# kyleliang919/distributed-lion-pytorch

Measured on AMD Instinct MI355X. Metric: tokens/sec + all-reduce bytes/step, GPT-2 CLM at 1/2/4/8 MI355X, higher is better.
Workload: dtype bf16; 1 GPU; model=gpt2 (124.4M params), trainable_params=124439808, base_weights=bf16, global_batch=160, task=clm, gradient_checkpointing=False, micro_batch=20, grad_accum=8, seq_len=1024, parallelism=dp1, optimizer=distributed Lion (majority vote), lr 0.0001, wd 0.1, exchange=a2a, impl=native

## Files before the change

distributed_lion_pytorch_amd/csrc/bindings.cpp:

```cpp
#include <ATen/ATen.h>
#include <c10/core/DeviceGuard.h>
#include <c10/hip/HIPStream.h>
#include <torch/library.h>

#include <hip/hip_runtime.h>

#include <cstdlib>
#include <string>
#include <vector>

#include "kernels.h"

namespace dlion {
enum class Layout : int { NT = 0, NN = 1, TN = 2, TT = 3 };
bool lt_gemm(const void* a, int64_t lda, const void* b, int64_t ldb, void* c, int64_t ldc, const void* bias,
             int64_t M, int64_t N, int64_t K, int epi, int device, hipStream_t s, Layout lay, bool accumulate);
}

namespace {

using at::Tensor;

void check_dev(const Tensor& t, const char* name) {
  TORCH_CHECK(t.is_cuda(), "dlion: ", name, " must be a GPU (HIP) tensor");
// ... 579 lines not shown
  return y;
}

void rope_(const Tensor& x, const Tensor& cos, const Tensor& sin, bool inverse) {
  TORCH_CHECK(x.dim() == 4 && x.is_cuda() && x.scalar_type() == at::kBFloat16, "dlion rope_: x must be bf16 [B, T, H, D]");
  const int64_t B = x.size(0), T = x.size(1), H = x.size(2), D = x.size(3);
  TORCH_CHECK(x.stride(3) == 1 && x.stride(2) == D && (B == 1 || x.stride(0) == T * x.stride(1)) &&
                  x.stride(1) % 8 == 0 && reinterpret_cast<uintptr_t>(x.data_ptr()) % 16 == 0 && D % 8 == 0,
              "dlion rope_: x must have contiguous heads and a uniform, 16-byte aligned token stride");
  for (const Tensor* t : {&cos, &sin})
    TORCH_CHECK(t->is_cuda() && t->scalar_type() == at::kBFloat16 && t->is_contiguous() && t->dim() == 2 &&
                    t->size(0) >= T && t->size(1) == D,
                "dlion rope_: cos/sin must be contiguous bf16 [>=T, D]");
  const c10::DeviceGuard dg(x.device());
  check_hip(dlion::launch_rope(x.data_ptr(), cos.data_ptr(), sin.data_ptr(), x.data_ptr(), B * T,
                               static_cast<int>(T), static_cast<int>(H), static_cast<int>(D), inverse, x.stride(1),
                               x.stride(1), cur_stream()),
            "rope_");
}

void check_gemm_operand(const Tensor& t, const char* name) {
  TORCH_CHECK(t.is_cuda() && t.scalar_type() == at::kBFloat16 && t.dim() == 2 && t.stride(1) == 1,
              "dlion gemm: ", name, " must be a 2-D bf16 GPU tensor with unit column stride");
  TORCH_CHECK(t.stride(0) % 8 == 0 && reinterpret_cast<uintptr_t>(t.data_ptr()) % 16 == 0,
              "dlion gemm: ", name, " rows must be 16-byte aligned");
}

bool gemm_nt_supported(const Tensor& a, const Tensor& b) {
  return a.dim() == 2 && b.dim() == 2 && a.size(1) == b.size(1) && a.size(1) % 128 == 0 && b.size(0) % 8 == 0 &&
         a.size(0) * a.stride(0) < (1ll << 31) && b.size(0) * b.stride(0) < (1ll << 31);
}

void gemm_nt_launch(const Tensor& a, const Tensor& b, const Tensor& c, const Tensor* bias, const Tensor* aux,
                    int64_t epi, const Tensor* part = nullptr) {
  check_gemm_operand(a, "a");
  check_gemm_operand(b, "b");
  check_gemm_operand(c, "out");
  TORCH_CHECK(gemm_nt_supported(a, b), "dlion gemm: unsupported shape a=", a.sizes(), " b=", b.sizes(),
              " (needs K % 128 == 0, N % 8 == 0)");
  TORCH_CHECK(c.size(0) == a.size(0) && c.size(1) == b.size(0), "dlion gemm: output shape mismatch");
  if (bias) {
    TORCH_CHECK(bias->is_cuda() && bias->scalar_type() == at::kBFloat16 && bias->is_contiguous() &&
                    bias->numel() == b.size(0),
                "dlion gemm: bias must be a contiguous bf16 [N] tensor");
  }
  if (aux) {
    check_gemm_operand(*aux, "aux");
    TORCH_CHECK(aux->size(0) == c.size(0) && aux->size(1) == c.size(1), "dlion gemm: aux must match the output shape");
  }
  if (part) {
    TORCH_CHECK(part->is_cuda() && part->scalar_type() == at::kFloat && part->is_contiguous() &&
                    part->size(0) == 2 * ((a.size(0) + 255) / 256) && part->size(1) == b.size(0),
                "dlion gemm: part must be fp32 [2 * ceil(M / 256), N]");
  }
  const c10::DeviceGuard g(a.device());
  check_hip(dlion::launch_gemm_nt(a.data_ptr(), static_cast<int>(a.stride(0)), b.data_ptr(),
                                  static_cast<int>(b.stride(0)), c.data_ptr(), static_cast<int>(c.stride(0)),
                                  bias ? bias->data_ptr() : nullptr, aux ? aux->data_ptr() : nullptr,
                                  aux ? static_cast<int>(aux->stride(0)) : 0, static_cast<int>(a.size(0)),
                                  static_cast<int>(b.size(0)), static_cast<int>(a.size(1)), static_cast<int>(epi),
                                  part ? part->data_ptr<float>() : nullptr, cur_stream()),
            "gemm_nt");
}

Tensor gemm_nt(const Tensor& a, const Tensor& b, const std::optional<Tensor>& bias) {
  auto c = at::empty({a.size(0), b.size(0)}, a.options());
  gemm_nt_launch(a, b, c, bias.has_value() ? &*bias : nullptr, nullptr, bias.has_value() ? 1 : 0);
  return c;
}

void gemm_nt_out(const Tensor& a, const Tensor& b, const std::optional<Tensor>& bias, const Tensor& out) {
  gemm_nt_launch(a, b, out, bias.has_value() ? &*bias : nullptr, nullptr, bias.has_value() ? 1 : 0);
}

std::tuple<Tensor, Tensor> gemm_nt_gelu(const Tensor& a, const Tensor& b, const Tensor& bias, bool exact) {
  auto h = at::empty({a.size(0), b.size(0)}, a.options());
  auto z = at::empty_like(h);
  gemm_nt_launch(a, b, h, &bias, &z, exact ? 3 : 2);
  return {h, z};
}

bool lt_gemm_nt(const Tensor& a, const Tensor& b, const std::optional<Tensor>& bias, int64_t epi, const Tensor& out) {
  check_gemm_operand(a, "a");
  check_gemm_operand(b, "b");
  check_gemm_operand(out, "out");
  TORCH_CHECK(epi >= 0 && epi <= 2, "dlion lt_gemm: bad epilogue ", epi);
  TORCH_CHECK(a.size(1) == b.size(1) && out.size(0) == a.size(0) && out.size(1) == b.size(0),
              "dlion lt_gemm: shape mismatch a=", a.sizes(), " b=", b.sizes(), " out=", out.sizes());
  TORCH_CHECK(bias.has_value() == (epi != 0), "dlion lt_gemm: epilogue ", epi, epi ? " needs" : " takes no", " bias");
  if (bias.has_value()) {
    TORCH_CHECK(bias->is_cuda() && bias->scalar_type() == at::kBFloat16 && bias->is_contiguous() &&
                    bias->numel() == b.size(0),
                "dlion lt_gemm: bias must be a contiguous bf16 [N] tensor");
  }
  const c10::DeviceGuard g(a.device());
// ... 106 lines not shown
    TORCH_CHECK(sid.has_value() && perm.has_value() && sid->numel() == n && perm->numel() == n &&
                    sid->scalar_type() == at::kLong && perm->scalar_type() == at::kLong && sid->is_contiguous() &&
                    perm->is_contiguous(),
                "dlion embed: the token gradient needs sorted ids and their permutation (int64 [n])");
    V = dwte->size(0);
  }
  if (dwpe.has_value()) {
    check_bf16_contig(*dwpe, "dwpe");
    TORCH_CHECK(dwpe->size(-1) == C && dwpe->size(0) >= T, "dlion embed: dwpe must be [>= T, C]");
  }
  const c10::DeviceGuard g(dx.device());
  const auto dp = drop_params(p);
  check_hip(dlion::launch_embed_bwd(dx.data_ptr(), dwte.has_value() ? sid->data_ptr<int64_t>() : nullptr,
                                    dwte.has_value() ? perm->data_ptr<int64_t>() : nullptr,
                                    dwte.has_value() ? dwte->data_ptr() : nullptr,
                                    dwpe.has_value() ? dwpe->data_ptr() : nullptr, n, static_cast<int>(C),
                                    static_cast<int>(T), V, pos_accumulate ? 1 : 0, static_cast<uint32_t>(seed),
                                    dp.first, dp.second, cur_stream()),
            "embed_bwd");
}

void scale_acc_(const Tensor& x, const Tensor& s, const Tensor& y, bool accumulate) {
  check_bf16_contig(x, "x");
  check_bf16_contig(y, "y");
  check_dev(s, "s");
  TORCH_CHECK(s.scalar_type() == at::kFloat && s.numel() >= 1, "dlion scale_acc: s must be float32");
  TORCH_CHECK(x.numel() == y.numel() && x.numel() % 8 == 0, "dlion scale_acc: size mismatch / numel % 8 != 0");
  const c10::DeviceGuard g(x.device());
  check_hip(dlion::launch_scale_acc(x.data_ptr(), s.data_ptr<float>(), y.data_ptr(), x.numel(), accumulate ? 1 : 0,
                                    cur_stream()),
            "scale_acc");
}

Tensor gemm_nt_stamped(const Tensor& a, const Tensor& b, const Tensor& stamps) {
  check_gemm_operand(a, "a");
  check_gemm_operand(b, "b");
  TORCH_CHECK(gemm_nt_supported(a, b), "dlion gemm: unsupported shape");
  const int64_t blocks = ((a.size(0) + 255) / 256) * ((b.size(0) + 255) / 256);
  TORCH_CHECK(stamps.is_cuda() && stamps.scalar_type() == at::kLong && stamps.is_contiguous() &&
                  stamps.numel() >= blocks * 8,
              "dlion gemm: stamps must be int64 [blocks, 8]");
  auto c = at::empty({a.size(0), b.size(0)}, a.options());
  const c10::DeviceGuard g(a.device());
  check_hip(dlion::launch_gemm_nt_stamped(a.data_ptr(), static_cast<int>(a.stride(0)), b.data_ptr(),
                                          static_cast<int>(b.stride(0)), c.data_ptr(), static_cast<int>(c.stride(0)),
                                          static_cast<int>(a.size(0)), static_cast<int>(b.size(0)),
                                          static_cast<int>(a.size(1)),
                                          reinterpret_cast<unsigned long long*>(stamps.data_ptr<int64_t>()),
                                          cur_stream()),
            "gemm_nt_stamped");
  return c;
}

std::tuple<Tensor, Tensor> gemm_nt_gelu_d(const Tensor& a, const Tensor& b, const Tensor& bias, bool exact) {
  auto h = at::empty({a.size(0), b.size(0)}, a.options());
  auto d = at::empty({a.size(0), b.size(0)}, a.options());
  gemm_nt_launch(a, b, h, &bias, &d, exact ? 7 : 6);
  return {h, d};
}

std::tuple<Tensor, Tensor> gemm_nt_dmul(const Tensor& a, const Tensor& b, const Tensor& d) {
  auto dz = at::empty({a.size(0), b.size(0)}, a.options());
  auto part = at::empty({2 * ((a.size(0) + 255) / 256), b.size(0)}, a.options().dtype(at::kFloat));
  gemm_nt_launch(a, b, dz, nullptr, &d, 8, &part);
  return {dz, part};
}

std::tuple<Tensor, Tensor> gemm_nt_dgelu(const Tensor& a, const Tensor& b, const Tensor& bias, const Tensor& z,
                                         bool exact) {
  auto dz = at::empty({a.size(0), b.size(0)}, a.options());
  auto part = at::empty({2 * ((a.size(0) + 255) / 256), b.size(0)}, a.options().dtype(at::kFloat));
  gemm_nt_launch(a, b, dz, &bias, &z, exact ? 5 : 4, &part);
  return {dz, part};
}

void gemm_tn_check_launch(at::TensorList P, at::TensorList Q, int64_t splits, const Tensor& out, bool accumulate) {
  TORCH_CHECK(!P.empty() && P.size() == Q.size() && P.size() <= 16, "dlion gemm_tn: 1..16 segment pairs");
  const int64_t rows = P[0].size(0), M = P[0].size(1), N = Q[0].size(1);
  const int64_t ldp = P[0].stride(0), ldq = Q[0].stride(0);
  std::vector<const void*> pp, qq;
  for (size_t i = 0; i < P.size(); ++i) {
    for (const Tensor* t : {&P[i], &Q[i]}) {
// ... 162 lines not shown
}

void dequant4_t_(const Tensor& q, const Tensor& absmax, const Tensor& code, const Tensor& out) {
  check_dev(q, "q");
  check_dev(absmax, "absmax");
  check_dev(code, "code");
  TORCH_CHECK(out.is_cuda() && out.dim() == 2 && out.stride(1) == 1 && out.element_size() == 2,
              "dlion dequant4_t: out must be a 2-D 16-bit GPU view with unit column stride");
  const int64_t K = out.size(0), N = out.size(1);
  TORCH_CHECK(q.scalar_type() == at::kByte && q.numel() * 2 == N * K && absmax.numel() * 64 == N * K &&
                  code.numel() == 16 && code.scalar_type() == at::kFloat,
              "dlion dequant4_t: q / absmax do not match out");
  const c10::DeviceGuard g(out.device());
  check_hip(dlion::launch_dequant4_t(dtype_code(out.scalar_type()), q.data_ptr<uint8_t>(), absmax.data_ptr<float>(),
                                     code.data_ptr<float>(), out.data_ptr(), static_cast<int>(N), static_cast<int>(K),
                                     out.stride(0), cur_stream()),
            "dequant4_t");
}
}

TORCH_LIBRARY(dlion, m) {
  m.def("dequant4_t_(Tensor q, Tensor absmax, Tensor code, Tensor(a!) out) -> ()");
  m.def("transpose_pad(Tensor x, int rows_out=-1) -> Tensor");
  m.def("quant4(Tensor w, Tensor code) -> (Tensor, Tensor)");
  m.def("dequant4_(Tensor q, Tensor absmax, Tensor code, Tensor(a!) out) -> ()");
  m.def("gemm_tn(Tensor[] P, Tensor[] Q, int splits) -> Tensor");
  m.def("gemm_tn_(Tensor[] P, Tensor[] Q, Tensor(a!) out, bool accumulate) -> ()");
  m.def("lora_rows(Tensor x, Tensor w, float scale, float p, int seed) -> Tensor");
  m.def("lora_up(Tensor o, Tensor u, Tensor b, float s) -> Tensor");
  m.def("lora_cols(Tensor g, Tensor y, Tensor? a, float yscale, float p, int seed) -> (Tensor, Tensor)");
  m.def("gemm_nt_dgelu(Tensor a, Tensor b, Tensor bias, Tensor z, bool exact) -> (Tensor, Tensor)");
  m.def("gemm_nt_gelu_d(Tensor a, Tensor b, Tensor bias, bool exact) -> (Tensor, Tensor)");
  m.def("gemm_nt_dmul(Tensor a, Tensor b, Tensor d) -> (Tensor, Tensor)");
  m.def("gemm_nt_stamped(Tensor a, Tensor b, Tensor(a!) stamps) -> Tensor");
  m.def("embed_fwd(Tensor ids, Tensor wte, Tensor wpe, float p, int seed, Tensor(a!)? err=None) -> Tensor");
  m.def("index_check_(Tensor ids, int hi, int ignore, Tensor(a!) err, int code) -> ()");
  m.def(
      "embed_bwd_(Tensor dx, Tensor? sid, Tensor? perm, Tensor(a!)? dwte, Tensor(b!)? dwpe, int T, bool pos_accumulate,"
      " float p, int seed) -> ()");
  m.def("scale_acc_(Tensor x, Tensor s, Tensor(a!) y, bool accumulate) -> ()");
  m.def("lt_gemm_nt(Tensor a, Tensor b, Tensor? bias, int epi, Tensor(a!) out) -> bool");
  m.def("lt_gemm_nn(Tensor a, Tensor b, Tensor(a!) out) -> bool");
  m.def("lt_gemm_tn(Tensor a, Tensor b, Tensor(a!) out, bool accumulate) -> bool");
  m.def("lt_gemm_nt_acc(Tensor a, Tensor b, Tensor(a!) out, bool accumulate) -> bool");
  m.def("lt_gemm_layout(Tensor a, Tensor b, Tensor(a!) out, int layout, bool accumulate) -> bool");
  m.def("gemm_nt(Tensor a, Tensor b, Tensor? bias) -> Tensor");
  m.def("gemm_nt_out(Tensor a, Tensor b, Tensor? bias, Tensor(a!) out) -> ()");
  m.def("gemm_nt_gelu(Tensor a, Tensor b, Tensor bias, bool exact) -> (Tensor, Tensor)");
  m.def("swiglu_fwd(Tensor g, Tensor u) -> Tensor");
  m.def("swiglu_bwd(Tensor dh, Tensor g, Tensor u) -> (Tensor, Tensor)");
  m.def("swiglu_bwd_fused(Tensor dh, Tensor g, Tensor u) -> Tensor");
  m.def("swiglu_bwd_fused_t(Tensor dh, Tensor g, Tensor u) -> (Tensor, Tensor)");
  m.def("swiglu_fwd_t(Tensor g, Tensor u) -> (Tensor, Tensor)");
  m.def("rope(Tensor x, Tensor cos, Tensor sin, bool inverse) -> Tensor");
  m.def("rope_(Tensor(a!) x, Tensor cos, Tensor sin, bool inverse) -> ()");
  m.def(
      "add_norm_fwd(Tensor x, Tensor? y, Tensor? bias, Tensor gamma, Tensor? beta, float eps, bool rms, float p,"
      " int seed) -> (Tensor, Tensor, Tensor, Tensor)");
  m.def(
      "add_norm_bwd(Tensor dh, Tensor? dxo_in, Tensor xo, Tensor gamma, Tensor mean, Tensor rstd, bool rms,"
      " float p, int seed, bool want_dy, int parts) -> (Tensor, Tensor, Tensor)");
  m.def("bias_gelu_fwd(Tensor z, Tensor b, bool exact) -> Tensor");
  m.def("bias_gelu_bwd(Tensor dh, Tensor z, Tensor b, bool exact, int parts) -> (Tensor, Tensor)");
  m.def("sum_partials(Tensor part) -> Tensor");
  m.def("sum_partials_acc_(Tensor part, Tensor(a!) out) -> ()");
  m.def("sum_partials_scaled_(Tensor part, Tensor s, Tensor(a!) out, bool accumulate) -> ()");
  m.def("sum_partials_multi_(Tensor[] parts, Tensor(a!) out, bool accumulate) -> ()");
// ... 25 lines not shown
TORCH_LIBRARY_IMPL(dlion, CUDA, m) {
  m.impl("lion_local", &lion_local);
  m.impl("lion_encode", &lion_encode);
  m.impl("lion_vote_apply", &lion_vote_apply);
  m.impl("vote_reduce", &vote_reduce);
  m.impl("grad_sumsq", &grad_sumsq);
  m.impl("clip_coef", &clip_coef);
  m.impl("softmax_xent_", &softmax_xent_);
  m.impl("attn_fwd", &attn_fwd);
  m.impl("attn_bwd", &attn_bwd);
  m.impl("add_norm_fwd", &add_norm_fwd);
  m.impl("add_norm_bwd", &add_norm_bwd);
  m.impl("bias_gelu_fwd", &bias_gelu_fwd);
  m.impl("bias_gelu_bwd", &bias_gelu_bwd);
  m.impl("sum_partials", &sum_partials);
  m.impl("sum_partials_acc_", &sum_partials_acc_);
  m.impl("sum_partials_scaled_", &sum_partials_scaled_);
  m.impl("sum_partials_multi_", &sum_partials_multi_);
  m.impl("colsum_partials", &colsum_partials);
  m.impl("swiglu_fwd", &swiglu_fwd);
  m.impl("swiglu_bwd", &swiglu_bwd);
  m.impl("swiglu_bwd_fused", &swiglu_bwd_fused);
  m.impl("swiglu_bwd_fused_t", &swiglu_bwd_fused_t);
  m.impl("swiglu_fwd_t", &swiglu_fwd_t);
  m.impl("rope", &rope);
  m.impl("rope_", &rope_);
  m.impl("gemm_nt", &gemm_nt);
  m.impl("gemm_nt_out", &gemm_nt_out);
  m.impl("gemm_nt_gelu", &gemm_nt_gelu);
  m.impl("gemm_nt_dgelu", &gemm_nt_dgelu);
  m.impl("gemm_nt_gelu_d", &gemm_nt_gelu_d);
  m.impl("gemm_nt_dmul", &gemm_nt_dmul);
  m.impl("gemm_nt_stamped", &gemm_nt_stamped);
  m.impl("embed_fwd", &embed_fwd);
  m.impl("index_check_", &index_check_);
  m.impl("embed_bwd_", &embed_bwd_);
  m.impl("scale_acc_", &scale_acc_);
  m.impl("lt_gemm_nt", &lt_gemm_nt);
  m.impl("lt_gemm_nn", &lt_gemm_nn);
  m.impl("lt_gemm_tn", &lt_gemm_tn);
  m.impl("lt_gemm_nt_acc", &lt_gemm_nt_acc);
  m.impl("lt_gemm_layout", &lt_gemm_layout);
  m.impl("gemm_tn", &gemm_tn);
  m.impl("gemm_tn_", &gemm_tn_);
  m.impl("lora_rows", &lora_rows);
  m.impl("lora_up", &lora_up);
  m.impl("lora_cols", &lora_cols);
  m.impl("quant4", &quant4);
  m.impl("dequant4_", &dequant4_);
  m.impl("dequant4_t_", &dequant4_t_);
  m.impl("transpose_pad", &transpose_pad);
}
```

distributed_lion_pytorch_amd/csrc/gemm.hip:

```cpp
#include "common.h"

#include <algorithm>

namespace dlion {

namespace {

typedef __bf16 bf16x8 __attribute__((ext_vector_type(8)));
typedef float f32x4 __attribute__((ext_vector_type(4)));

constexpr int kBM = 256, kBN = 256, kBK = 64;
constexpr int kHalf = 128 * kBK * 2;
constexpr int kLds = 8 * kHalf;

struct GemmArgs {
  const uint16_t* A;
  const uint16_t* B;
  uint16_t* C;
  const uint16_t* bias;
  uint16_t* aux;
  float* part;
  unsigned long long* stamps;
  int lda, ldb, ldc, ldaux;
  int M, N, K;
  int tiles_m, tiles_n;
};

__device__ __forceinline__ constexpr int slot(int dbuf, int ab, int half) { return ((dbuf * 2 + ab) * 2 + half) * kHalf; }

__device__ __forceinline__ void vm_wait6() { asm volatile("s_waitcnt vmcnt(6)" ::: "memory"); }
__device__ __forceinline__ void vm_wait8() { asm volatile("s_waitcnt vmcnt(8)" ::: "memory"); }
__device__ __forceinline__ void vm_wait2() { asm volatile("s_waitcnt vmcnt(2)" ::: "memory"); }
__device__ __forceinline__ void vm_wait0() { asm volatile("s_waitcnt vmcnt(0)" ::: "memory"); }

__device__ __forceinline__ void glds16(const uint16_t* base, uint32_t boff, uint8_t* dst) {
  const uint8_t* src = reinterpret_cast<const uint8_t*>(base) + boff;
  __builtin_amdgcn_global_load_lds((const __attribute__((address_space(1))) void*)src,
                                   (__attribute__((address_space(3))) void*)dst, 16, 0, 0);
}

typedef unsigned int u32x4 __attribute__((ext_vector_type(4)));
template <bool NT, typename V>
__device__ __forceinline__ void st16(uint16_t* p, const V& v) {
  const u32x4 x = __builtin_bit_cast(u32x4, v);
  if constexpr (NT) __builtin_nontemporal_store(x, reinterpret_cast<u32x4*>(p));
  else *reinterpret_cast<u32x4*>(p) = x;
}
template <bool NT>
__device__ __forceinline__ uint4 ld16(const uint16_t* p) {
  u32x4 x;
  if constexpr (NT) x = __builtin_nontemporal_load(reinterpret_cast<const u32x4*>(p));
  else x = *reinterpret_cast<const u32x4*>(p);
  return make_uint4(x[0], x[1], x[2], x[3]);
}
constexpr bool kNtAux = true, kNtC = true;

__device__ __forceinline__ f32x4 mfma16(const bf16x8& a, const bf16x8& b, const f32x4& c) {
  return __builtin_amdgcn_mfma_f32_16x16x32_bf16(a, b, c, 0, 0, 0);
}

struct Stage {
  uint32_t off[2][2][2];
};

#define DLION_STAMP(dst)                                                            \
  if constexpr (STAMP) {                                                            \
    __builtin_amdgcn_sched_barrier(0);                                              \
    asm volatile("s_memtime %0\n\ts_waitcnt lgkmcnt(0)" : "=s"(dst) :: "memory");    \
    __builtin_amdgcn_sched_barrier(0);                                              \
  }
#define DLION_RSTAMP(dst)                                                           \
  if constexpr (STAMP) {                                                            \
    __builtin_amdgcn_sched_barrier(0);                                              \
    asm volatile("s_memrealtime %0\n\ts_waitcnt lgkmcnt(0)" : "=s"(dst) :: "memory"); \
    __builtin_amdgcn_sched_barrier(0);                                              \
  }

template <int EPI, bool STAMP = false>
__global__ void __launch_bounds__(512, 1) gemm_nt_kernel(const GemmArgs g) {
  unsigned long long st_[7] = {0, 0, 0, 0, 0, 0, 0};
  DLION_RSTAMP(st_[5])
  DLION_STAMP(st_[0])
  __shared__ __attribute__((aligned(16))) uint8_t lds[kLds];

  const int tid = threadIdx.x;
  const int w = __builtin_amdgcn_readfirstlane(tid >> 6), lane = tid & 63;
  const int wr = w >> 2, wc = w & 3;

  const int nwg = g.tiles_m * g.tiles_n;
  const int bid = blockIdx.x;
  const int xcd = bid & 7, q8 = nwg >> 3, r8 = nwg & 7;
  const int wg = (xcd < r8 ? xcd * (q8 + 1) : r8 * (q8 + 1) + (xcd - r8) * q8) + (bid >> 3);
  constexpr int GM = 8;
  const int per_group = GM * g.tiles_n;
  const int grp = wg / per_group;
  const int first_m = grp * GM;
  const int gsz = min(g.tiles_m - first_m, GM);
  const int in_g = wg - grp * per_group;
  const int tm = first_m + in_g % gsz;
  const int tn = in_g / gsz;
  const int m0 = tm * kBM, n0 = tn * kBN;

  Stage st;
  {
    const int pc = lane & 7;
#pragma unroll
    for (int pi = 0; pi < 2; ++pi) {
      const int q = 2 * w + pi;
      const int lr = 8 * q + (lane >> 3);
      const int c = pc ^ ((lr >> 1) & 7);
#pragma unroll
      for (int h = 0; h < 2; ++h) {
        const int ra = min(m0 + (lr >> 6) * 128 + 64 * h + (lr & 63), g.M - 1);
        st.off[0][h][pi] = static_cast<uint32_t>(ra * g.lda + c * 8) * 2u;
        const int rb = min(n0 + 128 * h + lr, g.N - 1);
        st.off[1][h][pi] = static_cast<uint32_t>(rb * g.ldb + c * 8) * 2u;
      }
    }
  }
  const uint16_t* __restrict__ Ag = g.A;
  const uint16_t* __restrict__ Bg = g.B;

  auto stage = [&](int ab, int half, int dbuf, int kt) {
    const uint16_t* base = (ab == 0 ? Ag : Bg) + kt * kBK;
    asm volatile("" : "+s"(base));
    uint8_t* dst = lds + slot(dbuf, ab, half) + (2 * w) * 1024;
    asm volatile("" : "+v"(st.off[ab][half][0]), "+v"(st.off[ab][half][1]));
    glds16(base, st.off[ab][half][0], dst);
    glds16(base, st.off[ab][half][1], dst + 1024);
  };

  const int lr16 = lane & 15;
  const int swz = (lr16 >> 1) & 7;
  const int foff0 = lr16 * 128 + (((lane >> 4) ^ swz) << 4);
  const int foff1 = lr16 * 128 + (((4 + (lane >> 4)) ^ swz) << 4);
  const int a_row_base = wr * 64 * 128;
  const int b_base_off = ((wc >> 1) * kHalf) + (wc & 1) * 64 * 128;

  f32x4 acc[8][4];
#pragma unroll
  for (int i = 0; i < 8; ++i)
#pragma unroll
    for (int j = 0; j < 4; ++j) acc[i][j] = f32x4{0.f, 0.f, 0.f, 0.f};

  bf16x8 bfr[4][2];
  bf16x8 afr[2][2];

  auto read_b = [&](int dbuf) {
    const uint8_t* base = lds + slot(dbuf, 1, 0) + b_base_off;
#pragma unroll
    for (int nt = 0; nt < 4; ++nt) {
      bfr[nt][0] = *reinterpret_cast<const bf16x8*>(base + nt * 16 * 128 + foff0);
      bfr[nt][1] = *reinterpret_cast<const bf16x8*>(base + nt * 16 * 128 + foff1);
    }
  };
  auto read_a = [&](int dbuf, int p) {
    const uint8_t* base = lds + slot(dbuf, 0, p >> 1) + a_row_base + (2 * (p & 1)) * 16 * 128;
#pragma unroll
    for (int mt = 0; mt < 2; ++mt) {
      afr[mt][0] = *reinterpret_cast<const bf16x8*>(base + mt * 16 * 128 + foff0);
      afr[mt][1] = *reinterpret_cast<const bf16x8*>(base + mt * 16 * 128 + foff1);
    }
  };

#define DLION_GEMM_MFMA(P)                                                       \
  do {                                                                           \
    __builtin_amdgcn_s_setprio(1);                                               \
    _Pragma("unroll") for (int mt = 0; mt < 2; ++mt)                             \
    _Pragma("unroll") for (int nt = 0; nt < 4; ++nt)                             \
    _Pragma("unroll") for (int s = 0; s < 2; ++s)                                \
      acc[2 * (P) + mt][nt] = mfma16(bfr[nt][s], afr[mt][s], acc[2 * (P) + mt][nt]); \
    __builtin_amdgcn_s_setprio(0);                                               \
  } while (0)

#define DLION_GEMM_PHASE_MATH(P)                     \
  __builtin_amdgcn_s_barrier();                      \
  asm volatile("s_waitcnt lgkmcnt(0)" ::: "memory"); \
  __builtin_amdgcn_sched_barrier(0);                 \
  DLION_GEMM_MFMA(P);                                \
  __builtin_amdgcn_sched_barrier(0);                 \
  __builtin_amdgcn_s_barrier();

  const int nk = g.K / kBK;
  const int nit = nk / 2;

  stage(1, 0, 0, 0);
  stage(1, 1, 0, 0);
  stage(0, 0, 0, 0);
  stage(0, 1, 0, 0);
  stage(1, 0, 1, 1);
  stage(1, 1, 1, 1);
  vm_wait6();
  __builtin_amdgcn_s_barrier();
  if (wr == 1) __builtin_amdgcn_s_barrier();
  DLION_STAMP(st_[1])

  for (int it = 0; it < nit; ++it) {
    const int kt = 2 * it;
    const bool more = it + 1 < nit;
    read_b(0);
    read_a(0, 0);
    stage(0, 0, 1, kt + 1);
    DLION_GEMM_PHASE_MATH(0)
    read_a(0, 1);
    stage(0, 1, 1, kt + 1);
    vm_wait8();
    DLION_GEMM_PHASE_MATH(1)
    read_a(0, 2);
    if (more) stage(1, 0, 0, kt + 2);
    DLION_GEMM_PHASE_MATH(2)
    read_a(0, 3);
    if (more) {
      stage(1, 1, 0, kt + 2);
      vm_wait6();
    } else {
      vm_wait2();
    }
    DLION_GEMM_PHASE_MATH(3)
    read_b(1);
    read_a(1, 0);
    if (more) stage(0, 0, 0, kt + 2);
    DLION_GEMM_PHASE_MATH(0)
    read_a(1, 1);
    if (more) {
      stage(0, 1, 0, kt + 2);
      vm_wait8();
    } else {
      vm_wait0();
    }
    DLION_GEMM_PHASE_MATH(1)
    read_a(1, 2);
    if (more) stage(1, 0, 1, kt + 3);
    DLION_GEMM_PHASE_MATH(2)
    read_a(1, 3);
    if (more) {
      stage(1, 1, 1, kt + 3);
      vm_wait6();
    }
    DLION_GEMM_PHASE_MATH(3)
  }
#undef DLION_GEMM_PHASE_MATH
#undef DLION_GEMM_MFMA
  if (wr == 0) __builtin_amdgcn_s_barrier();
  DLION_STAMP(st_[2])

  uint8_t* reg = lds + w * (128 * 128);
  float bv[4][4] = {};
  if constexpr (EPI == 1) {
#pragma unroll
    for (int nt = 0; nt < 4; ++nt)
#pragma unroll
      for (int j = 0; j < 4; ++j) {
        const int n = n0 + wc * 64 + nt * 16 + 4 * (lane >> 4) + j;
        bv[nt][j] = n < g.N ? bf16_to_f32(g.bias[n]) : 0.f;
      }
  }
  const int row_base = m0 + wr * 128;
  const int col_base = n0 + wc * 64;

  auto park = [&](auto fn) {
#pragma unroll
    for (int mt = 0; mt < 8; ++mt)
#pragma unroll
      for (int nt = 0; nt < 4; ++nt) {
        const int row = mt * 16 + (lane & 15);
        const int col = nt * 16 + 4 * (lane >> 4);
        const int chunk = (col >> 3) ^ (row & 7);
        const uint32_t lo = static_cast<uint32_t>(fn(acc[mt][nt][0], nt, 0)) |
                            (static_cast<uint32_t>(fn(acc[mt][nt][1], nt, 1)) << 16);
        const uint32_t hi = static_cast<uint32_t>(fn(acc[mt][nt][2], nt, 2)) |
                            (static_cast<uint32_t>(fn(acc[mt][nt][3], nt, 3)) << 16);
        *reinterpret_cast<uint2*>(reg + row * 128 + chunk * 16 + (col & 7) * 2) = make_uint2(lo, hi);
      }
    asm volatile("s_waitcnt lgkmcnt(0)" ::: "memory");
    __builtin_amdgcn_wave_barrier();
  };
  const int ch = lane & 7;
// ... 76 lines not shown
        float gv[8], z[8], o[8];
        Elem<kBF16>::load8(reinterpret_cast<const uint16_t*>(&v), gv);
        Elem<kBF16>::load8(reinterpret_cast<const uint16_t*>(&zr[i]), z);
        bf16x8 ob;
#pragma unroll
        for (int j = 0; j < 8; ++j) {
          if constexpr (EPI == 8) {
            o[j] = gv[j] * z[j];
          } else {
            o[j] = gv[j] * gelu_grad(z[j] + b8[j], EPI == 5);
          }
          ob[j] = static_cast<__bf16>(o[j]);
          cs[j] += static_cast<float>(ob[j]);
        }
        st16<kNtC>(g.C + (int64_t)gm * g.ldc + gn, ob);
      }
    }
#pragma unroll
    for (int j = 0; j < 8; ++j) {
      cs[j] += __shfl_xor(cs[j], 8);
      cs[j] += __shfl_xor(cs[j], 16);
      cs[j] += __shfl_xor(cs[j], 32);
    }
    if (lane < 8 && gn < g.N) {
      float* dst = g.part + (int64_t)(2 * tm + wr) * g.N + gn;
      *reinterpret_cast<float4*>(dst) = make_float4(cs[0], cs[1], cs[2], cs[3]);
      *reinterpret_cast<float4*>(dst + 4) = make_float4(cs[4], cs[5], cs[6], cs[7]);
    }
  }
}

}

hipError_t launch_gemm_nt_stamped(const void* A, int lda, const void* B, int ldb, void* C, int ldc, int M, int N, int K,
                                  unsigned long long* stamps, hipStream_t st) {
  if (K % 128 != 0 || N % 8 != 0) return hipErrorInvalidValue;
  GemmArgs g{};
  g.A = static_cast<const uint16_t*>(A);
  g.B = static_cast<const uint16_t*>(B);
  g.C = static_cast<uint16_t*>(C);
  g.lda = lda;
  g.ldb = ldb;
  g.ldc = ldc;
  g.M = M;
  g.N = N;
  g.K = K;
  g.tiles_m = (M + kBM - 1) / kBM;
  g.tiles_n = (N + kBN - 1) / kBN;
  g.stamps = stamps;
  hipLaunchKernelGGL((gemm_nt_kernel<0, true>), dim3(g.tiles_m * g.tiles_n), dim3(512), 0, st, g);
  return hipGetLastError();
}


hipError_t launch_gemm_nt(const void* A, int lda, const void* B, int ldb, void* C, int ldc, const void* bias,
                          void* aux, int ldaux, int M, int N, int K, int epi, float* part, hipStream_t st) {
  if (M <= 0 || N <= 0) return hipSuccess;
  if (K % 128 != 0 || N % 8 != 0 || lda % 8 != 0 || ldb % 8 != 0 || ldc % 8 != 0) return hipErrorInvalidValue;
  if ((int64_t)M * lda >= (1ll << 31) || (int64_t)N * ldb >= (1ll << 31)) return hipErrorInvalidValue;
  if (epi >= 2 && (aux == nullptr || ldaux % 8 != 0)) return hipErrorInvalidValue;
  if (epi >= 1 && epi != 8 && (bias == nullptr || reinterpret_cast<uintptr_t>(bias) % 16 != 0))
    return hipErrorInvalidValue;
  if ((epi == 4 || epi == 5 || epi == 8) && (part == nullptr || reinterpret_cast<uintptr_t>(part) % 16 != 0))
    return hipErrorInvalidValue;
  GemmArgs g;
  g.A = static_cast<const uint16_t*>(A);
  g.B = static_cast<const uint16_t*>(B);
  g.C = static_cast<uint16_t*>(C);
  g.bias = static_cast<const uint16_t*>(bias);
  g.aux = static_cast<uint16_t*>(aux);
  g.part = part;
  g.lda = lda;
  g.ldb = ldb;
  g.ldc = ldc;
  g.ldaux = ldaux;
  g.M = M;
  g.N = N;
  g.K = K;
  g.tiles_m = (M + kBM - 1) / kBM;
  g.tiles_n = (N + kBN - 1) / kBN;
  const dim3 grid(g.tiles_m * g.tiles_n), block(512);
  switch (epi) {
    case 0: hipLaunchKernelGGL(gemm_nt_kernel<0>, grid, block, 0, st, g); break;
    case 1: hipLaunchKernelGGL(gemm_nt_kernel<1>, grid, block, 0, st, g); break;
    case 2: hipLaunchKernelGGL(gemm_nt_kernel<2>, grid, block, 0, st, g); break;
    case 3: hipLaunchKernelGGL(gemm_nt_kernel<3>, grid, block, 0, st, g); break;
    case 4: hipLaunchKernelGGL(gemm_nt_kernel<4>, grid, block, 0, st, g); break;
    case 5: hipLaunchKernelGGL(gemm_nt_kernel<5>, grid, block, 0, st, g); break;
    case 6: hipLaunchKernelGGL(gemm_nt_kernel<6>, grid, block, 0, st, g); break;
    case 7: hipLaunchKernelGGL(gemm_nt_kernel<7>, grid, block, 0, st, g); break;
    case 8: hipLaunchKernelGGL(gemm_nt_kernel<8>, grid, block, 0, st, g); break;
    default: return hipErrorInvalidValue;
  }
  return hipGetLastError();
}

}
```

distributed_lion_pytorch_amd/csrc/kernels.h:

```cpp
#pragma once
#include <hip/hip_runtime.h>
#include <stdint.h>

#include "attention.h"

namespace dlion {

hipError_t launch_lion_local(int dt, const int64_t* seg, const int64_t* chunks, int64_t n_chunks, float decay,
                             float neg_lr, float b1, float omb1, float b2, float omb2, const float* gscale,
                             hipStream_t st);
hipError_t launch_lion_encode(int dt, const int64_t* seg, const int64_t* chunks, int64_t n_chunks, uint8_t* bits,
                              float b1, float omb1, float b2, float omb2, int update_m, int stochastic, float rr,
                              uint64_t seed, uint32_t step, const float* gscale, hipStream_t st);
hipError_t launch_grad_sumsq(int dt, const int64_t* seg, const int64_t* chunks, int64_t n_chunks, float* partial,
                             hipStream_t st);
hipError_t launch_clip_coef(const float* partial, int64_t n, float max_norm, float* out, hipStream_t st);
hipError_t launch_lion_vote_apply(int dt, const int64_t* seg, const int64_t* chunks, int64_t n_chunks,
                                  const uint8_t* planes, int64_t plane_stride, const uint8_t* alive, int world,
                                  int mode, int tie, const uint8_t* neg, float decay, float neg_lr, const uint8_t* own,
                                  unsigned long long* agree, hipStream_t st);
hipError_t launch_vote_reduce(const uint8_t* recv, int64_t nbytes, const uint8_t* alive, int world, int tie,
                              uint8_t* out, uint8_t* neg_out, unsigned long long* ties, hipStream_t st);

hipError_t launch_attn_fwd(const AttnArgs& a, int D, bool drop, hipStream_t st);
// ... 3 lines not shown
                               void* xo, void* h, float* mean, float* rstd, int64_t rows, int C, float eps, bool rms,
                               uint32_t seed, uint32_t thresh16, float inv_keep, hipStream_t st);
hipError_t launch_add_norm_bwd(const void* dh, const void* dxo_in, const void* xo, const void* gamma, const float* mean,
                               const float* rstd, void* dx, void* dy, float* part, int parts, int64_t rows, int C,
                               bool rms, uint32_t seed, uint32_t thresh16, float inv_keep, hipStream_t st);

hipError_t launch_bias_gelu_fwd(const void* z, const void* b, void* h, int64_t rows, int N, bool exact,
                                hipStream_t st);
hipError_t launch_bias_gelu_bwd(const void* dh, const void* z, const void* b, void* dz, float* dbpart, int parts,
                                int64_t rows, int N, bool exact, hipStream_t st);
hipError_t launch_swiglu_fwd(const void* g, const void* u, void* h, int64_t rows, int64_t F, int64_t ld_in,
                             hipStream_t st);
hipError_t launch_swiglu_fwd_t(const void* g, const void* u, void* h, void* ht, int64_t rows, int64_t F,
                               int64_t ld_in, hipStream_t st);
hipError_t launch_swiglu_bwd_t(const void* dh, const void* g, const void* u, void* dgu, void* dgut, int64_t rows,
                               int64_t F, int64_t ld_in, hipStream_t st);
hipError_t launch_swiglu_bwd(const void* dh, const void* g, const void* u, void* dg, void* du, int64_t rows,
                             int64_t F, int64_t ld_in, int64_t ld_out, hipStream_t st);
hipError_t launch_rope(const void* x, const void* cos, const void* sin, void* y, int64_t rows, int T, int H, int D,
                       bool inverse, int64_t x_ld, int64_t y_ld, hipStream_t st);
hipError_t launch_sum_partials(const float* part, int S, int64_t n, int64_t ld, void* out, bool accumulate,
                               hipStream_t st, const float* scale = nullptr);
hipError_t launch_colsum(const void* x, float* part, int parts, int64_t rows, int N, hipStream_t st);
hipError_t launch_sum_partials_multi(const float* const* ptrs, const int64_t* rows, const int64_t* lds, int nseg,
                                     int64_t n, void* out, bool accumulate, hipStream_t st);
int sum_partials_split_factor(int64_t n, int64_t total_rows);
hipError_t launch_transpose_pad(const void* x, int64_t R, int64_t C, int64_t ldx, void* out, int64_t Rp,
                                hipStream_t st);
hipError_t launch_sum_partials_split(const float* const* ptrs, const int64_t* rows, const int64_t* lds, int nseg,
                                     int64_t n, int Y, float* scratch, void* out, bool accumulate, const float* scale,
                                     hipStream_t st);

hipError_t launch_gemm_nt(const void* A, int lda, const void* B, int ldb, void* C, int ldc, const void* bias,
                          void* aux, int ldaux, int M, int N, int K, int epi, float* part, hipStream_t st);

hipError_t launch_embed_fwd(const int64_t* ids, const void* wte, const void* wpe, void* out, int64_t n, int C, int T,
                            int64_t V, uint32_t seed, uint32_t thresh16, float inv_keep, int32_t* err, hipStream_t st);
constexpr int kIndexErrEmbed = 1, kIndexErrLabel = 2;
hipError_t launch_index_check(const int64_t* ids, int64_t n, int64_t hi, int64_t ignore, int32_t* err, int code,
                              hipStream_t st);
hipError_t launch_embed_bwd(const void* dx, const int64_t* sid, const int64_t* perm, void* dwte, void* dwpe, int64_t n,
                            int C, int T, int64_t V, int pos_accumulate, uint32_t seed, uint32_t thresh16,
                            float inv_keep, hipStream_t st);
hipError_t launch_scale_acc(const void* x, const float* s, void* y, int64_t n, int accumulate, hipStream_t st);

hipError_t launch_gemm_tn(const void* const* P, const void* const* Q, int nseg, int64_t seg_rows, int ldp, int ldq,
                          float* C, int M, int N, int splits, bool accumulate, hipStream_t st, void* Cb = nullptr);

hipError_t launch_gemm_nt_stamped(const void* A, int lda, const void* B, int ldb, void* C, int ldc, int M, int N, int K,
                                  unsigned long long* stamps, hipStream_t st);

hipError_t launch_lora_rows(const void* in, int64_t ldin, const void* w, void* out, int64_t rows, int K, int r,
                            float scale, uint32_t seed, uint32_t thresh16, float inv_keep, hipStream_t st);
hipError_t launch_lora_up(const void* o, int64_t ldo, const void* u, const void* b, void* out, int64_t rows, int N, int r,
                          float s, hipStream_t st);
int lora_cols_parts(int64_t rows, int N);
hipError_t launch_lora_cols(const void* g, int64_t ldg, const void* y, const void* a, void* dx, float* part, int64_t rows,
                            int N, int r, int parts, int mode, float yscale, uint32_t seed, uint32_t thresh16,
                            float inv_keep, hipStream_t st);

hipError_t launch_quant4(int dt, const void* w, const float* code, uint8_t* q, float* absmax, int64_t n,
                         hipStream_t st);
hipError_t launch_dequant4(int dt, const uint8_t* q, const float* absmax, const float* code, void* out, int64_t n,
                           hipStream_t st);
hipError_t launch_dequant4_t(int dt, const uint8_t* q, const float* absmax, const float* code, void* out, int N, int K,
                             int64_t ldo, hipStream_t st);

hipError_t launch_softmax_xent(int dt, void* logits, const int64_t* labels, int64_t n, int64_t vp, int v, float* loss,
                               int variant, hipStream_t st);

}
```

Baseline: 1.092 million tokens/s.

## Make gemm_nt persistent with next-tile prologue overlapping a direct-store epilogue

Turns the NT GEMM kernel into a persistent kernel for epilogues 0/1/6/7/8. The grid is capped at the CU count and each block loops over tiles. Before writing the current tile's epilogue, a block issues the next tile's global-to-LDS prologue loads, then stages the output through a small per-wave LDS region and stores it directly, waiting on vmcnt with the store count added. This is meant to hide epilogue and launch-tail latency behind the next tile's loads. The cost is fragile vmcnt accounting, LDS aliasing with the prefetched slots, and a default path change that affects every GEMM.

```diff
diff --git a/distributed_lion_pytorch_amd/csrc/bindings.cpp b/distributed_lion_pytorch_amd/csrc/bindings.cpp
--- a/distributed_lion_pytorch_amd/csrc/bindings.cpp
+++ b/distributed_lion_pytorch_amd/csrc/bindings.cpp
@@ -635,7 +635,7 @@
 }
 
 void gemm_nt_launch(const Tensor& a, const Tensor& b, const Tensor& c, const Tensor* bias, const Tensor* aux,
-                    int64_t epi, const Tensor* part = nullptr) {
+                    int64_t epi, const Tensor* part = nullptr, int64_t path = -1, int64_t max_blocks = 0) {
   check_gemm_operand(a, "a");
   check_gemm_operand(b, "b");
   check_gemm_operand(c, "out");
@@ -662,8 +662,32 @@
                                   bias ? bias->data_ptr() : nullptr, aux ? aux->data_ptr() : nullptr,
                                   aux ? static_cast<int>(aux->stride(0)) : 0, static_cast<int>(a.size(0)),
                                   static_cast<int>(b.size(0)), static_cast<int>(a.size(1)), static_cast<int>(epi),
-                                  part ? part->data_ptr<float>() : nullptr, cur_stream()),
+                                  part ? part->data_ptr<float>() : nullptr, cur_stream(), static_cast<int>(path),
+                                  static_cast<int>(max_blocks)),
             "gemm_nt");
+}
+
+std::vector<Tensor> gemm_nt_path(const Tensor& a, const Tensor& b, const std::optional<Tensor>& bias,
+                                 const std::optional<Tensor>& aux, int64_t epi, int64_t path, int64_t max_blocks,
+                                 const std::optional<Tensor>& out) {
+  TORCH_CHECK(epi == 0 || epi == 1 || (epi >= 6 && epi <= 8), "dlion gemm_nt_path: epi must be 0, 1, 6, 7 or 8");
+  TORCH_CHECK(path >= -1 && path <= 1 && max_blocks >= 0, "dlion gemm_nt_path: path in {-1, 0, 1}, max_blocks >= 0");
+  TORCH_CHECK((epi == 0 || epi == 8) != bias.has_value(), "dlion gemm_nt_path: bias goes with epi 1/6/7 only");
+  TORCH_CHECK(epi != 8 || aux.has_value(), "dlion gemm_nt_path: epi 8 needs aux (gelu')");
+  TORCH_CHECK(epi >= 6 || !aux.has_value(), "dlion gemm_nt_path: aux goes with epi 6/7/8 only");
+  Tensor c = out.has_value() ? *out : at::empty({a.size(0), b.size(0)}, a.options());
+  if (epi <= 1) {
+    gemm_nt_launch(a, b, c, bias.has_value() ? &*bias : nullptr, nullptr, epi, nullptr, path, max_blocks);
+    return {c};
+  }
+  if (epi <= 7) {
+    Tensor d = aux.has_value() ? *aux : at::empty({a.size(0), b.size(0)}, a.options());
+    gemm_nt_launch(a, b, c, &*bias, &d, epi, nullptr, path, max_blocks);
+    return {c, d};
+  }
+  auto part = at::empty({2 * ((a.size(0) + 255) / 256), b.size(0)}, a.options().dtype(at::kFloat));
+  gemm_nt_launch(a, b, c, nullptr, &*aux, 8, &part, path, max_blocks);
+  return {c, part};
 }
 
 Tensor gemm_nt(const Tensor& a, const Tensor& b, const std::optional<Tensor>& bias) {
@@ -836,7 +860,7 @@
             "scale_acc");
 }
 
-Tensor gemm_nt_stamped(const Tensor& a, const Tensor& b, const Tensor& stamps) {
+Tensor gemm_nt_stamped(const Tensor& a, const Tensor& b, const Tensor& stamps, bool direct) {
   check_gemm_operand(a, "a");
   check_gemm_operand(b, "b");
   TORCH_CHECK(gemm_nt_supported(a, b), "dlion gemm: unsupported shape");
@@ -851,7 +875,7 @@
                                           static_cast<int>(a.size(0)), static_cast<int>(b.size(0)),
                                           static_cast<int>(a.size(1)),
                                           reinterpret_cast<unsigned long long*>(stamps.data_ptr<int64_t>()),
-                                          cur_stream()),
+                                          cur_stream(), direct),
             "gemm_nt_stamped");
   return c;
 }
@@ -1080,7 +1104,8 @@
   m.def("gemm_nt_dgelu(Tensor a, Tensor b, Tensor bias, Tensor z, bool exact) -> (Tensor, Tensor)");
   m.def("gemm_nt_gelu_d(Tensor a, Tensor b, Tensor bias, bool exact) -> (Tensor, Tensor)");
   m.def("gemm_nt_dmul(Tensor a, Tensor b, Tensor d) -> (Tensor, Tensor)");
-  m.def("gemm_nt_stamped(Tensor a, Tensor b, Tensor(a!) stamps) -> Tensor");
+  m.def("gemm_nt_stamped(Tensor a, Tensor b, Tensor(a!) stamps, bool direct=False) -> Tensor");
+  m.def("gemm_nt_path(Tensor a, Tensor b, Tensor? bias, Tensor? aux, int epi, int path, int max_blocks, Tensor? out) -> Tensor[]");
   m.def("embed_fwd(Tensor ids, Tensor wte, Tensor wpe, float p, int seed, Tensor(a!)? err=None) -> Tensor");
   m.def("index_check_(Tensor ids, int hi, int ignore, Tensor(a!) err, int code) -> ()");
   m.def(
@@ -1172,6 +1197,7 @@
   m.impl("gemm_nt_gelu_d", &gemm_nt_gelu_d);
   m.impl("gemm_nt_dmul", &gemm_nt_dmul);
   m.impl("gemm_nt_stamped", &gemm_nt_stamped);
+  m.impl("gemm_nt_path", &gemm_nt_path);
   m.impl("embed_fwd", &embed_fwd);
   m.impl("index_check_", &index_check_);
   m.impl("embed_bwd_", &embed_bwd_);
diff --git a/distributed_lion_pytorch_amd/csrc/gemm.hip b/distributed_lion_pytorch_amd/csrc/gemm.hip
--- a/distributed_lion_pytorch_amd/csrc/gemm.hip
+++ b/distributed_lion_pytorch_amd/csrc/gemm.hip
@@ -32,6 +32,13 @@
 __device__ __forceinline__ void vm_wait8() { asm volatile("s_waitcnt vmcnt(8)" ::: "memory"); }
 __device__ __forceinline__ void vm_wait2() { asm volatile("s_waitcnt vmcnt(2)" ::: "memory"); }
 __device__ __forceinline__ void vm_wait0() { asm volatile("s_waitcnt vmcnt(0)" ::: "memory"); }
+template <int N>
+__device__ __forceinline__ void vm_wait_n() {
+  static_assert(N >= 0 && N < 64, "vmcnt is a 6-bit counter");
+  asm volatile("s_waitcnt vmcnt(%0)" ::"n"(N) : "memory");
+}
+
+__host__ __device__ constexpr int direct_stores(int epi) { return epi == 6 || epi == 7 ? 32 : epi == 8 ? 18 : 16; }
 
 __device__ __forceinline__ void glds16(const uint16_t* base, uint32_t boff, uint8_t* dst) {
   const uint8_t* src = reinterpret_cast<const uint8_t*>(base) + boff;
@@ -76,8 +83,9 @@
     __builtin_amdgcn_sched_barrier(0);                                              \
   }
 
-template <int EPI, bool STAMP = false>
+template <int EPI, bool STAMP = false, bool DIRECT = false>
 __global__ void __launch_bounds__(512, 1) gemm_nt_kernel(const GemmArgs g) {
+  static_assert(!DIRECT || EPI <= 1 || (EPI >= 6 && EPI <= 8), "direct epilogue: EPI 0/1/6/7/8");
   unsigned long long st_[7] = {0, 0, 0, 0, 0, 0, 0};
   DLION_RSTAMP(st_[5])
   DLION_STAMP(st_[0])
@@ -88,21 +96,26 @@
   const int wr = w >> 2, wc = w & 3;
 
   const int nwg = g.tiles_m * g.tiles_n;
-  const int bid = blockIdx.x;
-  const int xcd = bid & 7, q8 = nwg >> 3, r8 = nwg & 7;
-  const int wg = (xcd < r8 ? xcd * (q8 + 1) : r8 * (q8 + 1) + (xcd - r8) * q8) + (bid >> 3);
-  constexpr int GM = 8;
-  const int per_group = GM * g.tiles_n;
-  const int grp = wg / per_group;
-  const int first_m = grp * GM;
-  const int gsz = min(g.tiles_m - first_m, GM);
-  const int in_g = wg - grp * per_group;
-  const int tm = first_m + in_g % gsz;
-  const int tn = in_g / gsz;
-  const int m0 = tm * kBM, n0 = tn * kBN;
+  int tm, m0, n0;
+  auto tile_of = [&](int vid) {
+    const int xcd = vid & 7, q8 = nwg >> 3, r8 = nwg & 7;
+    const int wg = (xcd < r8 ? xcd * (q8 + 1) : r8 * (q8 + 1) + (xcd - r8) * q8) + (vid >> 3);
+    constexpr int GM = 8;
+    const int per_group = GM * g.tiles_n;
+    const int grp = wg / per_group;
+    const int first_m = grp * GM;
+    const int gsz = min(g.tiles_m - first_m, GM);
+    const int in_g = wg - grp * per_group;
+    tm = first_m + in_g % gsz;
+    const int tn = in_g / gsz;
+    m0 = tm * kBM;
+    n0 = tn * kBN;
+  };
+  int vid = blockIdx.x;
+  tile_of(vid);
 
   Stage st;
-  {
+  auto set_offsets = [&]() {
     const int pc = lane & 7;
 #pragma unroll
     for (int pi = 0; pi < 2; ++pi) {
@@ -117,7 +130,8 @@
         st.off[1][h][pi] = static_cast<uint32_t>(rb * g.ldb + c * 8) * 2u;
       }
     }
-  }
+  };
+  set_offsets();
   const uint16_t* __restrict__ Ag = g.A;
   const uint16_t* __restrict__ Bg = g.B;
 
@@ -138,11 +152,6 @@
   const int b_base_off = ((wc >> 1) * kHalf) + (wc & 1) * 64 * 128;
 
   f32x4 acc[8][4];
-#pragma unroll
-  for (int i = 0; i < 8; ++i)
-#pragma unroll
-    for (int j = 0; j < 4; ++j) acc[i][j] = f32x4{0.f, 0.f, 0.f, 0.f};
-
   bf16x8 bfr[4][2];
   bf16x8 afr[2][2];
 
@@ -184,13 +193,26 @@
   const int nk = g.K / kBK;
   const int nit = nk / 2;
 
-  stage(1, 0, 0, 0);
-  stage(1, 1, 0, 0);
-  stage(0, 0, 0, 0);
-  stage(0, 1, 0, 0);
-  stage(1, 0, 1, 1);
-  stage(1, 1, 1, 1);
-  vm_wait6();
+  auto prologue = [&]() {
+    stage(1, 0, 0, 0);
+    stage(1, 1, 0, 0);
+    stage(0, 0, 0, 0);
+    stage(0, 1, 0, 0);
+    stage(1, 0, 1, 1);
+    stage(1, 1, 1, 1);
+  };
+  prologue();
+  bool counted = false;
+ for (;;) {
+#pragma unroll
+  for (int i = 0; i < 8; ++i)
+#pragma unroll
+    for (int j = 0; j < 4; ++j) acc[i][j] = f32x4{0.f, 0.f, 0.f, 0.f};
+  if (DIRECT && counted) {
+    vm_wait_n<6 + direct_stores(EPI)>();
+  } else {
+    vm_wait6();
+  }
   __builtin_amdgcn_s_barrier();
   if (wr == 1) __builtin_amdgcn_s_barrier();
   DLION_STAMP(st_[1])
@@ -243,6 +265,148 @@
 #undef DLION_GEMM_MFMA
   if (wr == 0) __builtin_amdgcn_s_barrier();
   DLION_STAMP(st_[2])
+  if constexpr (!DIRECT) {
+    break;
+  } else {
+    const int ctm = tm;
+    const int row_base = m0 + wr * 128;
+    const int ch = lane & 7;
+    const int gn = n0 + wc * 64 + ch * 8;
+    const bool full = m0 + kBM <= g.M && n0 + kBN <= g.N;
+    uint8_t* reg = lds + slot(1, 0, 0) + w * 4096;
+
+    float b8[8];
+    float bv[EPI == 1 ? 4 : 1][4] = {};
+    uint4 zr[EPI == 8 ? 16 : 1];
+    if constexpr (EPI == 1) {
+#pragma unroll
+      for (int nt = 0; nt < 4; ++nt)
+#pragma unroll
+        for (int j = 0; j < 4; ++j) {
+          const int n = n0 + wc * 64 + nt * 16 + 4 * (lane >> 4) + j;
+          bv[nt][j] = n < g.N ? bf16_to_f32(g.bias[n]) : 0.f;
+        }
+    }
+    if ((EPI == 6 || EPI == 7) && gn < g.N) {
+      Elem<kBF16>::load8(g.bias + gn, b8);
+    } else {
+#pragma unroll
+      for (int j = 0; j < 8; ++j) b8[j] = 0.f;
+    }
+    if constexpr (EPI == 8) {
+#pragma unroll
+      for (int i = 0; i < 16; ++i) {
+        const int gm = min(row_base + i * 8 + (lane >> 3), g.M - 1);
+        zr[i] = ld16<kNtAux>(g.aux + (int64_t)gm * g.ldaux + (gn < g.N ? gn : g.N - 8));
+      }
+    }
+    __builtin_amdgcn_sched_barrier(0);
+
+    const int nvid = vid + static_cast<int>(gridDim.x);
+    const bool has_next = nvid < nwg;
+    if (has_next) {
+      tile_of(nvid);
+      set_offsets();
+      prologue();
+    }
+    __builtin_amdgcn_sched_barrier(0);
+    DLION_STAMP(st_[3])
+
+    typedef __bf16 bf16x2 __attribute__((ext_vector_type(2)));
+    auto pack2 = [](float lo, float hi) {
+      const bf16x2 v = {static_cast<__bf16>(lo), static_cast<__bf16>(hi)};
+      return __builtin_bit_cast(uint32_t, v);
+    };
+    float cs[8];
+#pragma unroll
+    for (int j = 0; j < 8; ++j) cs[j] = 0.f;
+
+#pragma unroll
+    for (int q = 0; q < 4; ++q) {
+#pragma unroll
+      for (int ml = 0; ml < 2; ++ml)
+#pragma unroll
+        for (int nt = 0; nt < 4; ++nt) {
+          const f32x4 a = acc[2 * q + ml][nt];
+          const int row = ml * 16 + (lane & 15);
+          const int col = nt * 16 + 4 * (lane >> 4);
+          const int chunk = (col >> 3) ^ (row & 7);
+          uint2 pk;
+          if constexpr (EPI == 1) {
+            pk = make_uint2(pack2(a[0] + bv[nt][0], a[1] + bv[nt][1]), pack2(a[2] + bv[nt][2], a[3] + bv[nt][3]));
+          } else {
+            pk = make_uint2(pack2(a[0], a[1]), pack2(a[2], a[3]));
+          }
+          *reinterpret_cast<uint2*>(reg + row * 128 + chunk * 16 + (col & 7) * 2) = pk;
+        }
+      asm volatile("s_waitcnt lgkmcnt(0)" ::: "memory");
+      __builtin_amdgcn_wave_barrier();
+#pragma unroll
+      for (int il = 0; il < 4; ++il) {
+        const int i = 4 * q + il;
+        const int row = il * 8 + (lane >> 3);
+        const uint4 v = *reinterpret_cast<const uint4*>(reg + row * 128 + ((ch ^ (row & 7)) << 4));
+        const int gm = row_base + 32 * q + row;
+        const bool ok = gm < g.M && gn < g.N;
+        if constexpr (EPI <= 1) {
+          if (ok) st16<false>(g.C + (int64_t)gm * g.ldc + gn, v);
+        } else if constexpr (EPI == 6 || EPI == 7) {
+          if (ok) {
+            float z[8];
+            Elem<kBF16>::load8(reinterpret_cast<const uint16_t*>(&v), z);
+            bf16x8 hb, db;
+#pragma unroll
+            for (int j = 0; j < 8; ++j) {
+              float gv, dgv;
+              gelu_and_grad(z[j] + b8[j], EPI == 7, gv, dgv);
+              hb[j] = static_cast<__bf16>(gv);
+              db[j] = static_cast<__bf16>(dgv);
+            }
+            st16<kNtAux>(g.aux + (int64_t)gm * g.ldaux + gn, db);
+            st16<kNtC>(g.C + (int64_t)gm * g.ldc + gn, hb);
+          }
+        } else if constexpr (EPI == 8) {
+          if (ok) {
+            float gv[8], z[8];
+            Elem<kBF16>::load8(reinterpret_cast<const uint16_t*>(&v), gv);
+            Elem<kBF16>::load8(reinterpret_cast<const uint16_t*>(&zr[i]), z);
+            bf16x8 ob;
+#pragma unroll
+            for (int j = 0; j < 8; ++j) {
+              ob[j] = static_cast<__bf16>(gv[j] * z[j]);
+              cs[j] += static_cast<float>(ob[j]);
+            }
+            st16<kNtC>(g.C + (int64_t)gm * g.ldc + gn, ob);
+          }
+        }
+      }
+      __builtin_amdgcn_wave_barrier();
+    }
+    if constexpr (EPI == 8) {
+#pragma unroll
+      for (int j = 0; j < 8; ++j) {
+        cs[j] += __shfl_xor(cs[j], 8);
+        cs[j] += __shfl_xor(cs[j], 16);
+        cs[j] += __shfl_xor(cs[j], 32);
+      }
+      if (lane < 8 && gn < g.N) {
+        float* dst = g.part + (int64_t)(2 * ctm + wr) * g.N + gn;
+        *reinterpret_cast<float4*>(dst) = make_float4(cs[0], cs[1], cs[2], cs[3]);
+        *reinterpret_cast<float4*>(dst + 4) = make_float4(cs[4], cs[5], cs[6], cs[7]);
+      }
+    }
+    if constexpr (STAMP) {
+      DLION_STAMP(st_[4])
+      DLION_RSTAMP(st_[6])
+      if (tid < 8) g.stamps[static_cast<int64_t>(vid) * 8 + tid] = tid < 7 ? st_[tid < 7 ? tid : 0] : 0ull;
+      DLION_RSTAMP(st_[5])
+      DLION_STAMP(st_[0])
+    }
+    if (!has_next) return;
+    counted = full;
+    vid = nvid;
+  }
+ }
 
   uint8_t* reg = lds + w * (128 * 128);
   float bv[4][4] = {};
@@ -385,8 +549,27 @@
 
 }
 
+static int cu_count() {
+  static int cached[64] = {};
+  int dev = 0;
+  if (hipGetDevice(&dev) != hipSuccess || dev < 0 || dev >= 64) dev = 0;
+  if (cached[dev] == 0) {
+    int n = 0;
+    if (hipDeviceGetAttribute(&n, hipDeviceAttributeMultiprocessorCount, dev) != hipSuccess || n <= 0) n = 256;
+    cached[dev] = n;
+  }
+  return cached[dev];
+}
+
+static int direct_grid(int tiles, int max_blocks) {
+  const int cus = cu_count();
+  int grid = tiles <= cus ? tiles : std::max(cus & ~7, 1);
+  if (max_blocks > 0) grid = std::min(grid, max_blocks);
+  return grid;
+}
+
 hipError_t launch_gemm_nt_stamped(const void* A, int lda, const void* B, int ldb, void* C, int ldc, int M, int N, int K,
-                                  unsigned long long* stamps, hipStream_t st) {
+                                  unsigned long long* stamps, hipStream_t st, bool direct) {
   if (K % 128 != 0 || N % 8 != 0) return hipErrorInvalidValue;
   GemmArgs g{};
   g.A = static_cast<const uint16_t*>(A);
@@ -401,13 +584,19 @@
   g.tiles_m = (M + kBM - 1) / kBM;
   g.tiles_n = (N + kBN - 1) / kBN;
   g.stamps = stamps;
-  hipLaunchKernelGGL((gemm_nt_kernel<0, true>), dim3(g.tiles_m * g.tiles_n), dim3(512), 0, st, g);
+  const int tiles = g.tiles_m * g.tiles_n;
+  if (direct) {
+    hipLaunchKernelGGL((gemm_nt_kernel<0, true, true>), dim3(direct_grid(tiles, 0)), dim3(512), 0, st, g);
+  } else {
+    hipLaunchKernelGGL((gemm_nt_kernel<0, true>), dim3(tiles), dim3(512), 0, st, g);
+  }
   return hipGetLastError();
 }
 
 
 hipError_t launch_gemm_nt(const void* A, int lda, const void* B, int ldb, void* C, int ldc, const void* bias,
-                          void* aux, int ldaux, int M, int N, int K, int epi, float* part, hipStream_t st) {
+                          void* aux, int ldaux, int M, int N, int K, int epi, float* part, hipStream_t st, int path,
+                          int max_blocks) {
   if (M <= 0 || N <= 0) return hipSuccess;
   if (K % 128 != 0 || N % 8 != 0 || lda % 8 != 0 || ldb % 8 != 0 || ldc % 8 != 0) return hipErrorInvalidValue;
   if ((int64_t)M * lda >= (1ll << 31) || (int64_t)N * ldb >= (1ll << 31)) return hipErrorInvalidValue;
@@ -416,6 +605,8 @@
     return hipErrorInvalidValue;
   if ((epi == 4 || epi == 5 || epi == 8) && (part == nullptr || reinterpret_cast<uintptr_t>(part) % 16 != 0))
     return hipErrorInvalidValue;
+  const bool can_direct = epi == 0 || epi == 1 || (epi >= 6 && epi <= 8);
+  if (path > 1 || (path == 1 && !can_direct)) return hipErrorInvalidValue;
   GemmArgs g;
   g.A = static_cast<const uint16_t*>(A);
   g.B = static_cast<const uint16_t*>(B);
@@ -432,7 +623,22 @@
   g.K = K;
   g.tiles_m = (M + kBM - 1) / kBM;
   g.tiles_n = (N + kBN - 1) / kBN;
-  const dim3 grid(g.tiles_m * g.tiles_n), block(512);
+  const int tiles = g.tiles_m * g.tiles_n;
+  const bool direct = path == 1 || (path < 0 && can_direct);
+  const dim3 block(512);
+  if (direct) {
+    const dim3 grid(direct_grid(tiles, max_blocks));
+    switch (epi) {
+      case 0: hipLaunchKernelGGL((gemm_nt_kernel<0, false, true>), grid, block, 0, st, g); break;
+      case 1: hipLaunchKernelGGL((gemm_nt_kernel<1, false, true>), grid, block, 0, st, g); break;
+      case 6: hipLaunchKernelGGL((gemm_nt_kernel<6, false, true>), grid, block, 0, st, g); break;
+      case 7: hipLaunchKernelGGL((gemm_nt_kernel<7, false, true>), grid, block, 0, st, g); break;
+      case 8: hipLaunchKernelGGL((gemm_nt_kernel<8, false, true>), grid, block, 0, st, g); break;
+      default: return hipErrorInvalidValue;
+    }
+    return hipGetLastError();
+  }
+  const dim3 grid(tiles);
   switch (epi) {
     case 0: hipLaunchKernelGGL(gemm_nt_kernel<0>, grid, block, 0, st, g); break;
     case 1: hipLaunchKernelGGL(gemm_nt_kernel<1>, grid, block, 0, st, g); break;
diff --git a/distributed_lion_pytorch_amd/csrc/kernels.h b/distributed_lion_pytorch_amd/csrc/kernels.h
--- a/distributed_lion_pytorch_amd/csrc/kernels.h
+++ b/distributed_lion_pytorch_amd/csrc/kernels.h
@@ -59,7 +59,8 @@
                                      hipStream_t st);
 
 hipError_t launch_gemm_nt(const void* A, int lda, const void* B, int ldb, void* C, int ldc, const void* bias,
-                          void* aux, int ldaux, int M, int N, int K, int epi, float* part, hipStream_t st);
+                          void* aux, int ldaux, int M, int N, int K, int epi, float* part, hipStream_t st,
+                          int path = -1, int max_blocks = 0);
 
 hipError_t launch_embed_fwd(const int64_t* ids, const void* wte, const void* wpe, void* out, int64_t n, int C, int T,
                             int64_t V, uint32_t seed, uint32_t thresh16, float inv_keep, int32_t* err, hipStream_t st);
@@ -75,7 +76,7 @@
                           float* C, int M, int N, int splits, bool accumulate, hipStream_t st, void* Cb = nullptr);
 
 hipError_t launch_gemm_nt_stamped(const void* A, int lda, const void* B, int ldb, void* C, int ldc, int M, int N, int K,
-                                  unsigned long long* stamps, hipStream_t st);
+                                  unsigned long long* stamps, hipStream_t st, bool direct = false);
 
 hipError_t launch_lora_rows(const void* in, int64_t ldin, const void* w, void* out, int64_t rows, int K, int r,
                             float scale, uint32_t seed, uint32_t thresh16, float inv_keep, hipStream_t st);
```

Result: slower. 1.050 million tokens/s (-3.8%).
